# ariana-spalter/human-robot-gym

Measured on AMD Instinct MI355X. Metric: env steps/sec (whole node), ReachHuman+shield 4096 envs, higher is better.
Workload: dtype f64

## Files before the change

human-robot-gym_amd/csrc/hrgym_device.h:

```cpp
#pragma once
#include <hip/hip_runtime.h>
#include <stdint.h>

#include "../../include/hrgym.h"
#include "../../include/hrgym_state.h"

#define NV HRG_NV
#define NARM HRG_NARM
#ifndef HRG_BOX
#define HRG_BOX 0
#endif
#ifndef HRG_LIFT
#define HRG_LIFT 0
#endif
#ifndef HRG_HANDOVER
#define HRG_HANDOVER 0
#endif
#ifndef HRG_STACK
#define HRG_STACK 0
#endif
#ifndef HRG_HULLS
#define HRG_HULLS 0
#endif
#ifndef HRG_HAMMER
#define HRG_HAMMER 0
#endif
#define HRG_BASE_TU (!HRG_BOX && !HRG_STACK && !HRG_HAMMER && !HRG_HULLS)
#define HRG_POSE_TABLE ((!HRG_BOX && !HRG_STACK && !HRG_HAMMER) || HRG_LIFT)
#define HRG_POSE_HCAP 0
#define HRG_POSE_SITE (6 * HRG_NHB)
#define HRG_POSE_ROOT (HRG_POSE_SITE + 3 * HRG_NHJ)
#define HRG_POSE_DIM (HRG_POSE_ROOT + 3)
#define NVT HRG_NVT
#if HRG_HAMMER
#define NVS HRG_NV_HAMMER
#define NCON_DYN HRG_NCON_DYN_HAMMER
#define HM_OB NV
#define HM_ON (NV + 6)
#define HM_OH (NV + 8)
#elif HRG_STACK
#define NVS HRG_NV_STACK
#define NCON_DYN HRG_NCON_DYN_STACK
#define NCUBE HRG_NCUBE
#elif HRG_BOX
#define NVS NVT
#define NCON_DYN HRG_NCON_DYN_BOX
#else
#define NVS NV
#define NCON_DYN HRG_NCON_DYN
#endif
#define BODY_BOX 100
#define DI __device__ __forceinline__
#ifndef HRG_MIN_WAVES
#define HRG_MIN_WAVES 4
#endif
#ifndef HRG_PHASE
#define HRG_PHASE __device__ __forceinline__
#endif
#define PH_DYNTERMS HRG_PHASE
#define PH_HUMAN HRG_PHASE
#define PH_SHIELD HRG_PHASE
#define PH_COLLIDE HRG_PHASE
#define PH_CLASSIFY HRG_PHASE
#define PH_DYNSTEP HRG_PHASE
#define HRG_PI 3.14159265358979323846
#define SIXTH (1.0 / 6.0)

#define GEOM_HUMAN0 HRG_NRCAP
#define GEOM_TABLE (HRG_NRCAP + HRG_NHB)
#define GEOM_FLOOR (GEOM_TABLE + 1)
#define GEOM_BOX (GEOM_FLOOR + 1)

#ifdef HRG_STAMPS
static __device__ unsigned long long g_stamps[32];
static __device__ unsigned long long g_stamps_slow[34];
static __device__ unsigned long long g_slow_thresh = ~0ull;
static __device__ unsigned long long g_envcyc[16384][3];
static __device__ unsigned long long g_envacc[16384][32];
__shared__ unsigned long long g_tbeg;
__shared__ unsigned long long g_acc[32];
__shared__ unsigned long long g_t0;
#define STAMP_NOW(var) do { __builtin_amdgcn_sched_barrier(0); asm volatile("s_memtime %0\n\ts_waitcnt lgkmcnt(0)" : "=s"(var) :: "memory"); __builtin_amdgcn_sched_barrier(0); } while (0)
#define STAMP_DECL
#define STAMP_INIT(lane) do { if ((lane) < 32) g_acc[lane] = 0; unsigned long long _t; STAMP_NOW(_t); g_t0 = _t; g_tbeg = _t; __syncthreads(); } while (0)
#define STAMP(k) do { unsigned long long _t; STAMP_NOW(_t); if (threadIdx.x == 0) { g_acc[k] += _t - g_t0; g_t0 = _t; } } while (0)
#define STAMP_FLUSH(lane)
#define COUNT(k, n) do { if (threadIdx.x == 0) g_acc[k] += (n); } while (0)
#define STAMP_FINAL(lane) do { __syncthreads(); if ((lane) < 32) atomicAdd(&g_stamps[lane], g_acc[lane]); { unsigned long long _te; STAMP_NOW(_te); if (_te - g_tbeg > g_slow_thresh) { if ((lane) < 32) atomicAdd(&g_stamps_slow[lane], g_acc[lane]); if ((lane) == 32) atomicAdd(&g_stamps_slow[32], 1ull); if ((lane) == 33) atomicAdd(&g_stamps_slow[33], _te - g_tbeg); } } if ((lane) < 32 && blockIdx.x < 16384) g_envacc[blockIdx.x][lane] = g_acc[lane]; if ((lane) == 0 && blockIdx.x < 16384) { unsigned long long _t; STAMP_NOW(_t); g_envcyc[blockIdx.x][0] = g_tbeg; g_envcyc[blockIdx.x][1] = _t; unsigned _hw, _xcc; asm volatile("s_getreg_b32 %0, hwreg(HW_REG_HW_ID)\n\ts_getreg_b32 %1, hwreg(HW_REG_XCC_ID)" : "=s"(_hw), "=s"(_xcc)); g_envcyc[blockIdx.x][2] = ((unsigned long long)_xcc << 32) | _hw; } } while (0)
#else
#define STAMP_DECL
#define STAMP_INIT(lane)
#define STAMP(k)
#define STAMP_FLUSH(lane)
#define COUNT(k, n)
#define STAMP_FINAL(lane)
#endif

struct DevModel {
  hrg_model_desc m;
  double Rbase[9];
  double Rq[NV][9];
  int32_t anc_mask[NV];
  int32_t hb_maxdepth;
  double sol_K, sol_Bd;
  double rcap_hl[HRG_NRCAP], hcap_hl[HRG_NHB];
  int32_t hb_njump;
  int32_t hb_jump[4][HRG_NHB];
  int32_t phase_mask;
  hrg_path brake_full;
  double brake_T, brake_ds;
  int32_t hc_n;
  int32_t hc_kind[HRG_NHCAP_MAX], hc_j1[HRG_NHCAP_MAX], hc_j2[HRG_NHCAP_MAX];
  double hc_th[HRG_NHCAP_MAX], hc_v[HRG_NHCAP_MAX], hc_a[HRG_NHCAP_MAX], hc_len[HRG_NHCAP_MAX];
  int32_t n_self;
  int32_t self_i[64], self_j[64];
  int32_t n_chk;
  int32_t chk_i[32], chk_j[32];
  hrg_clip_table clips;
  const double* pose_tab;
  const double* hull_dev;
  double hull_cen[HRG_NHULL][3];
  unsigned long long* mpr_fallback;
};

static inline void hull_centroids(const double* verts, const int32_t* off, double cen[HRG_NHULL][3]) {
  for (int h = 0; h < HRG_NHULL; h++) {
    double s[3] = {0, 0, 0};
    for (int i = off[h]; i < off[h + 1]; i++) for (int a = 0; a < 3; a++) s[a] += verts[3 * i + a];
    for (int a = 0; a < 3; a++) cen[h][a] = s[a] / (double)(off[h + 1] - off[h]);
  }
}

struct Contact {
  int32_t g1, g2, b1, b2;
  double dist, n[3], pos[3];
};

#define ROW_CON0 24
#define ROW_WELD0 (ROW_CON0 + 4 * NCON_DYN)
#if HRG_HAMMER
#define HROW_NFRIC 8
#define HROW_LIM0 9
#define HROW_NLIM 25
#define HROW_EQ0 27
#define HROW_CON0 36
#define HROW_NEQ 9
#define NROW 128
#elif HRG_STACK
#define SROW_WELD0 24
#define SROW_CON0 36
#define NROW HRG_NROW_STACK
#elif HRG_BOX && (HRG_HANDOVER || HRG_LIFT)
#define NROW (ROW_WELD0 + 6)
#else
#define NROW ROW_WELD0
#endif

struct GjkLds { double y[4][3], a[4][3], b[4][3], l[4], lam[4]; int ia[4], ib[4]; };
#if HRG_HULLS && HRG_BOX
struct MprLds { double v[5][3], a[5][3], b[5][3]; };
#endif
struct Lds {
  hrg_env_state st;
  double kR[NV][9], kp[NV][3], Sw[NV][3], Sv[NV][3], vw[NV][3], vv[NV][3];
  double M[NV * NV];
  double bias[NV], a0[NVS], Ma0[NVS], ctrl[NV], qacc[NVS], g[NVS], d[NVS];
#if HRG_BOX
  hrg_box_state bx;
  double bR[9];
  double bMr[9];
  double hand_q[4], hand_off[3];
  int palm_hit, palm_pad;
#if HRG_HANDOVER
  double hcap_keep[HRG_NHB][6];
#endif
#endif
  double act[NV];
  int acc_has_collision, acc_collision_type, acc_failsafe, acc_pad;
#if HRG_HAMMER
  hrg_hammer_state hm;
  double gR[2][9];
  double gc[HRG_HM_NGEOM][3];
  double nail_org[3], nail_axis[3];
  double Mb[64], fb[8];
  double Ihw[9], tauh[3];
  double nsG[(9 + 2 * NCON_DYN) * (10 + 2 * NCON_DYN) / 2];
  Contact con[NCON_DYN];
#elif HRG_STACK
  hrg_stack_state sk;
  Contact con[NCON_DYN];
#elif HRG_BOX
  Contact con[NCON_DYN];
#else
  Contact con[NCON_DYN];
#endif
  union {
    struct {
      double cq[NARM], cv[NARM], ca[NARM], qe[NARM];
      double scap[2][HRG_NSHIELD_RCAP][6];
      double rc[HRG_NSHIELD_RCAP][7];
      hrg_ltt cand;
    };
    struct {
      double F[NV][6];
    };
    struct {
      double hcap[HRG_NHB][6], rcapw[HRG_NRCAP][6];
      int hnear[HRG_NHB];
      double rcen[HRG_NRCAP][3];
#if HRG_HULLS && HRG_BOX
      union { GjkLds gjk; MprLds mpr; };
#elif HRG_HULLS
      GjkLds gjk;
#endif
#if HRG_STACK
      double cR[NCUBE][9];
#endif
    };
#if HRG_HAMMER
    struct {
      double Jc[4 * NCON_DYN + HROW_NEQ][NVS + 1], rg[NROW], rh[NROW];
    };
#elif HRG_STACK
    struct {
      double Jc[4 * NCON_DYN][21], rg[NROW], rh[NROW];
      int con_ca[NCON_DYN], con_cb[NCON_DYN], con_rob[NCON_DYN + 1];
    };
#else
    struct {
      double Jc[4 * NCON_DYN + (HRG_LIFT ? 6 : 0)][NVS + 1], rg[NROW], rh[NROW];
    };
#endif
  };
};

#ifndef HRG_WG_WAVES
#define HRG_WG_WAVES 1
#endif
#if HRG_WG_WAVES > 1
__shared__ Lds g_Lw[HRG_WG_WAVES];
#define g_L (g_Lw[__builtin_amdgcn_readfirstlane((int)(threadIdx.x >> 6))])
#else
__shared__ Lds g_L;
#endif
DI int hrg_lane() { return (int)(threadIdx.x & 63u); }
#define HRG_FAIR_SLOTS (8 * 8 * 2 * 16 * 4 * 8)
struct StepOrder { int32_t* buf; int32_t n; int32_t parity; int32_t* fair; };
DI int hrg_env() { return (int)blockIdx.x * HRG_WG_WAVES + (int)(threadIdx.x >> 6); }
// ... 634 lines not shown
```

human-robot-gym_amd/csrc/hrgym_hip.hip:

```cpp
#include <hip/hip_runtime.h>

#include <cmath>
#include <cstdio>
#include <cstring>
#include <cstdlib>
#include <memory>
#include <string>
#include <vector>

#include "hrgym_kernels.h"

template <class MD>
DI void impedance(const MD& m, double x0, double* imp) {
  const double d0 = m.solimp[0], dmax = m.solimp[1], width = m.solimp[2], mid = m.solimp[3], power = m.solimp[4];
  const double x = fabs(x0) / width;
  double y;
  if (x >= 1) y = 1;
  else if (x <= 0) y = 0;
  else if (x <= mid) { const double u = x / mid; y = u * u * mid; }
  else { const double u = (1 - x) / (1 - mid); y = 1 - u * u * (1 - mid); }
  (void)power;
  *imp = d0 + y * (dmax - d0);
}

// ... 2927 lines not shown
                                                                           int64_t env_id0, hrg_box_state* boxes);
extern "C" __attribute__((visibility("hidden"))) void hrg_lift_launch_step(int n_envs, hipStream_t st, const DevModel* dm, hrg_env_state* states, double* actions, float* obs, float* term_obs,
                                                                            float* reward, uint8_t* done, int32_t* info, double* dbg_r, double* dbg_h, int32_t* dbg_nh, int64_t env_id0,
                                                                            float* scratch_obs, hrg_box_state* boxes, StepOrder ord);
extern "C" __attribute__((visibility("hidden"))) void hrg_lift_launch_reset(int n_envs, hipStream_t st, const DevModel* dm, hrg_env_state* states, const uint8_t* mask, float* obs,
                                                                             int64_t env_id0, hrg_box_state* boxes);
#endif
#if HRG_BASE_TU
extern "C" __attribute__((visibility("hidden"))) void hrg_box_hull_launch_step(int n_envs, hipStream_t st, const DevModel* dm, hrg_env_state* states, double* actions, float* obs, float* term_obs,
                                                                                float* reward, uint8_t* done, int32_t* info, double* dbg_r, double* dbg_h, int32_t* dbg_nh, int64_t env_id0,
                                                                                float* scratch_obs, hrg_box_state* boxes, StepOrder ord);
extern "C" __attribute__((visibility("hidden"))) void hrg_box_hull_launch_reset(int n_envs, hipStream_t st, const DevModel* dm, hrg_env_state* states, const uint8_t* mask, float* obs,
                                                                                 int64_t env_id0, hrg_box_state* boxes);
extern "C" __attribute__((visibility("hidden"))) void hrg_hull_launch_step(int n_envs, hipStream_t st, const DevModel* dm, hrg_env_state* states, double* actions, float* obs, float* term_obs,
                                                                            float* reward, uint8_t* done, int32_t* info, double* dbg_r, double* dbg_h, int32_t* dbg_nh, int64_t env_id0,
                                                                            float* scratch_obs, StepOrder ord);
extern "C" __attribute__((visibility("hidden"))) void hrg_hull_launch_reset(int n_envs, hipStream_t st, const DevModel* dm, hrg_env_state* states, const uint8_t* mask, float* obs,
                                                                             int64_t env_id0);
#endif
#if HRG_HULLS && !HRG_BOX
extern "C" void hrg_hull_launch_step(int n_envs, hipStream_t st, const DevModel* dm, hrg_env_state* states, double* actions, float* obs, float* term_obs, float* reward, uint8_t* done,
                                     int32_t* info, double* dbg_r, double* dbg_h, int32_t* dbg_nh, int64_t env_id0, float* scratch_obs, StepOrder ord) {
  hipLaunchKernelGGL(hrg_step_kernel, HRG_LAUNCH_DIMS(n_envs), 0, st, dm, states, actions, obs, term_obs, reward, done, info, dbg_r, dbg_h, dbg_nh, env_id0, scratch_obs, (ObjState*)nullptr, n_envs, ord);
}
extern "C" void hrg_hull_launch_reset(int n_envs, hipStream_t st, const DevModel* dm, hrg_env_state* states, const uint8_t* mask, float* obs, int64_t env_id0) {
  hipLaunchKernelGGL(hrg_reset_kernel, HRG_LAUNCH_DIMS(n_envs), 0, st, dm, states, mask, obs, env_id0, (ObjState*)nullptr, n_envs);
}
#endif
#if HRG_HAMMER
extern "C" void hrg_hammer_launch_step(int n_envs, hipStream_t st, const DevModel* dm, hrg_env_state* states, double* actions, float* obs, float* term_obs, float* reward, uint8_t* done,
                                       int32_t* info, double* dbg_r, double* dbg_h, int32_t* dbg_nh, int64_t env_id0, float* scratch_obs, hrg_hammer_state* hammers, StepOrder ord) {
  hipLaunchKernelGGL(hrg_step_kernel, HRG_LAUNCH_DIMS(n_envs), 0, st, dm, states, actions, obs, term_obs, reward, done, info, dbg_r, dbg_h, dbg_nh, env_id0, scratch_obs, hammers, n_envs, ord);
}
extern "C" void hrg_hammer_launch_reset(int n_envs, hipStream_t st, const DevModel* dm, hrg_env_state* states, const uint8_t* mask, float* obs, int64_t env_id0, hrg_hammer_state* hammers) {
  hipLaunchKernelGGL(hrg_reset_kernel, HRG_LAUNCH_DIMS(n_envs), 0, st, dm, states, mask, obs, env_id0, hammers, n_envs);
}
#endif
#if HRG_STACK
extern "C" void hrg_stack_launch_step(int n_envs, hipStream_t st, const DevModel* dm, hrg_env_state* states, double* actions, float* obs, float* term_obs, float* reward, uint8_t* done,
                                      int32_t* info, double* dbg_r, double* dbg_h, int32_t* dbg_nh, int64_t env_id0, float* scratch_obs, hrg_stack_state* stacks, StepOrder ord) {
  hipLaunchKernelGGL(hrg_step_kernel, HRG_LAUNCH_DIMS(n_envs), 0, st, dm, states, actions, obs, term_obs, reward, done, info, dbg_r, dbg_h, dbg_nh, env_id0, scratch_obs, stacks, n_envs, ord);
}
extern "C" void hrg_stack_launch_reset(int n_envs, hipStream_t st, const DevModel* dm, hrg_env_state* states, const uint8_t* mask, float* obs, int64_t env_id0, hrg_stack_state* stacks) {
  hipLaunchKernelGGL(hrg_reset_kernel, HRG_LAUNCH_DIMS(n_envs), 0, st, dm, states, mask, obs, env_id0, stacks, n_envs);
}
#endif
#if HRG_BOX
extern "C" void hrg_box_launch_step(int n_envs, hipStream_t st, const DevModel* dm, hrg_env_state* states, double* actions, float* obs, float* term_obs, float* reward, uint8_t* done,
                                    int32_t* info, double* dbg_r, double* dbg_h, int32_t* dbg_nh, int64_t env_id0, float* scratch_obs, hrg_box_state* boxes, StepOrder ord) {
  hipLaunchKernelGGL(hrg_step_kernel, HRG_LAUNCH_DIMS(n_envs), 0, st, dm, states, actions, obs, term_obs, reward, done, info, dbg_r, dbg_h, dbg_nh, env_id0, scratch_obs, boxes, n_envs, ord);
}
extern "C" void hrg_box_launch_reset(int n_envs, hipStream_t st, const DevModel* dm, hrg_env_state* states, const uint8_t* mask, float* obs, int64_t env_id0, hrg_box_state* boxes) {
  hipLaunchKernelGGL(hrg_reset_kernel, HRG_LAUNCH_DIMS(n_envs), 0, st, dm, states, mask, obs, env_id0, boxes, n_envs);
}
#endif

#ifdef HRG_STAMPS
#if HRG_STACK
#define hrg_debug_stamps hrg_debug_stamps_stack
#elif HRG_HAMMER
#define hrg_debug_stamps hrg_debug_stamps_hammer
#elif HRG_BOX && HRG_HULLS
#define hrg_debug_stamps hrg_debug_stamps_box_hull
#elif HRG_HANDOVER
#define hrg_debug_stamps hrg_debug_stamps_ho
#elif HRG_LIFT
#define hrg_debug_stamps hrg_debug_stamps_lift
#elif HRG_BOX
#define hrg_debug_stamps hrg_debug_stamps_box
#elif HRG_HULLS
#define hrg_debug_stamps hrg_debug_stamps_hull
#endif
#if HRG_BASE_TU
extern "C" int hrg_debug_stamps_slow(double* out, unsigned long long thresh, int reset) {
  unsigned long long h[34];
  if (hipMemcpyFromSymbol(h, HIP_SYMBOL(g_stamps_slow), sizeof h) != hipSuccess) return -1;
  for (int i = 0; i < 34; i++) out[i] = (double)h[i];
  if (reset) { memset(h, 0, sizeof h); hipMemcpyToSymbol(HIP_SYMBOL(g_stamps_slow), h, sizeof h); }
  hipMemcpyToSymbol(HIP_SYMBOL(g_slow_thresh), &thresh, sizeof thresh);
  return 0;
}
#endif
extern "C" int hrg_debug_stamps(double* out, int reset) {
  unsigned long long h[32];
  if (hipMemcpyFromSymbol(h, HIP_SYMBOL(g_stamps), sizeof h) != hipSuccess) return -1;
  for (int i = 0; i < 32; i++) out[i] = (double)h[i];
  if (reset) { memset(h, 0, sizeof h); hipMemcpyToSymbol(HIP_SYMBOL(g_stamps), h, sizeof h); }
  return 0;
}
#if HRG_HAMMER
#define hrg_debug_envacc hrg_debug_envacc_hammer
#define hrg_debug_envcyc hrg_debug_envcyc_hammer
#elif HRG_STACK
#define hrg_debug_envacc hrg_debug_envacc_stack
#define hrg_debug_envcyc hrg_debug_envcyc_stack
#elif HRG_BOX && HRG_HULLS
#define hrg_debug_envacc hrg_debug_envacc_box_hull
#define hrg_debug_envcyc hrg_debug_envcyc_box_hull
#elif HRG_HANDOVER
#define hrg_debug_envacc hrg_debug_envacc_ho
#define hrg_debug_envcyc hrg_debug_envcyc_ho
#elif HRG_LIFT
#define hrg_debug_envacc hrg_debug_envacc_lift
#define hrg_debug_envcyc hrg_debug_envcyc_lift
#elif HRG_BOX
#define hrg_debug_envacc hrg_debug_envacc_box
#define hrg_debug_envcyc hrg_debug_envcyc_box
#elif HRG_HULLS
#define hrg_debug_envacc hrg_debug_envacc_hull
#define hrg_debug_envcyc hrg_debug_envcyc_hull
#endif
#if 1
extern "C" int hrg_debug_envacc(unsigned long long* out, int n) { return hipMemcpyFromSymbol(out, HIP_SYMBOL(g_envacc), sizeof(unsigned long long) * 32 * n) == hipSuccess ? 0 : -1; }
extern "C" int hrg_debug_envcyc(unsigned long long* out, int n) { return hipMemcpyFromSymbol(out, HIP_SYMBOL(g_envcyc), sizeof(unsigned long long) * 3 * n) == hipSuccess ? 0 : -1; }
#endif
#endif

#if HRG_BASE_TU

static thread_local std::string g_err;
static int fail(int code, const std::string& msg) { g_err = msg; return code; }
#define HIPCHK(x)                                                                                         \
  do {                                                                                                    \
    hipError_t _e = (x);                                                                                  \
    if (_e != hipSuccess) return fail(HRG_ERR_HIP, std::string(#x) + ": " + hipGetErrorString(_e));        \
  } while (0)

struct hrg_batch {
  int device = 0;
  int32_t n_envs = 0;
  int64_t env_id0 = 0;
  DevModel* d_model = nullptr;
  double* d_frames = nullptr;
  double* d_pose = nullptr;
  size_t pose_bytes = 0;
  double* d_hull = nullptr;
  bool hulls = false;
  unsigned long long* d_mpr_fallback = nullptr;
  hrg_env_state* d_states = nullptr;
  double* d_rcaps = nullptr;
  double* d_hcaps = nullptr;
  int32_t* d_nh = nullptr;
  float* d_scratch_obs = nullptr;
  hrg_box_state* d_boxes = nullptr;
  hrg_stack_state* d_stacks = nullptr;
  hrg_hammer_state* d_hammers = nullptr;
  int32_t* d_order = nullptr;
  int32_t parity = 0;
  int32_t task = HRG_TASK_REACH;
  bool timing = false;
  bool taps = false;
  std::vector<std::pair<hipEvent_t, hipEvent_t>> events;
  std::vector<std::pair<hipEvent_t, hipEvent_t>> pool;
};

static int32_t* fair_table(int device) {
  static int32_t* tab[64] = {nullptr};
  if (device < 0 || device >= 64) return nullptr;
  if (!tab[device]) {
    int32_t* p = nullptr;
    if (hipMalloc(&p, sizeof(int32_t) * HRG_FAIR_SLOTS) != hipSuccess) return nullptr;
    if (hipMemset(p, 0, sizeof(int32_t) * HRG_FAIR_SLOTS) != hipSuccess) { hipFree(p); return nullptr; }
    tab[device] = p;
  }
  return tab[device];
}

static bool hrg_task_uses_pose_table(int task) { return task == HRG_TASK_REACH || task == HRG_TASK_LIFTING; }

// ... 498 lines not shown
```

human-robot-gym_amd/csrc/hrgym_kernels.h:

```cpp
#pragma once
#include "hrgym_device.h"
#if HRG_HULLS
#include "hrgym_hull.h"
#endif

DI void robot_chain_fk(const DevModel* __restrict__ dm_, int lane, bool shield_on) {
  const ModelPtr dm = uniform_model(dm_);
  Lds& L = g_L;
  double* sc = &L.rc[0][0];
  if (lane < 3 * NARM && (lane >= 2 * NARM || shield_on)) {
    const int cfg = lane / NARM, i = lane - NARM * cfg;
    const double q = cfg == 0 ? L.cq[i] : (cfg == 1 ? L.qe[i] : L.st.qpos[i]);
    double sn, cs;
    sincos_small(q, &sn, &cs);
    sc[2 * lane] = sn; sc[2 * lane + 1] = cs;
  }
  wave_sync();
  if (lane < 9 && (lane >= 6 || shield_on)) {
    const auto& m = dm->m;
    const int cfg = lane / 3, row = lane - 3 * cfg;
    double r0 = dm->Rbase[3 * row], r1 = dm->Rbase[3 * row + 1], r2 = dm->Rbase[3 * row + 2];
    double p = m.base_pos[row];
#pragma unroll 1
    for (int i = 0; i < NARM; i++) {
      const double sn = sc[2 * (NARM * cfg + i)], cs = sc[2 * (NARM * cfg + i) + 1];
      p += r0 * m.body_pos[i][0] + r1 * m.body_pos[i][1] + r2 * m.body_pos[i][2];
      double n0 = 0, n1 = 0, n2 = 0;
      {
        const double ra[3] = {r0, r1, r2};
#pragma unroll
        for (int a = 0; a < 3; a++) {
          const double c0 = dm->Rq[i][3 * a], c1 = dm->Rq[i][3 * a + 1], c2 = dm->Rq[i][3 * a + 2];
          n0 += ra[a] * (cs * c0 + sn * c1);
          n1 += ra[a] * (cs * c1 - sn * c0);
          n2 += ra[a] * c2;
        }
      }
      r0 = n0; r1 = n1; r2 = n2;
      if (cfg == 2) {
        L.kR[i][3 * row] = r0; L.kR[i][3 * row + 1] = r1; L.kR[i][3 * row + 2] = r2;
        L.kp[i][row] = p;
      } else {
        L.scap[cfg][i][row] = p + (r0 * m.scap_p1[i][0] + r1 * m.scap_p1[i][1] + r2 * m.scap_p1[i][2]);
        L.scap[cfg][i][3 + row] = p + (r0 * m.scap_p2[i][0] + r1 * m.scap_p2[i][1] + r2 * m.scap_p2[i][2]);
        if (i == NARM - 1) {
          L.scap[cfg][NARM][row] = p + (r0 * m.scap_p1[NARM][0] + r1 * m.scap_p1[NARM][1] + r2 * m.scap_p1[NARM][2]);
          L.scap[cfg][NARM][3 + row] = p + (r0 * m.scap_p2[NARM][0] + r1 * m.scap_p2[NARM][1] + r2 * m.scap_p2[NARM][2]);
        }
      }
    }
    if (cfg == 2) {
#pragma unroll 1
      for (int f = 0; f < HRG_NFINGER; f++) {
        const int i = NARM + f;
        double l[3] = {0, 0, 0};
        {
          const double ra[3] = {r0, r1, r2};
#pragma unroll
          for (int a = 0; a < 3; a++)
#pragma unroll
            for (int b = 0; b < 3; b++) l[b] += ra[a] * dm->Rq[i][3 * a + b];
        }
        double pf = p + (r0 * m.body_pos[i][0] + r1 * m.body_pos[i][1] + r2 * m.body_pos[i][2]);
        const double axw = l[0] * m.jnt_axis[i][0] + l[1] * m.jnt_axis[i][1] + l[2] * m.jnt_axis[i][2];
        pf += axw * L.st.qpos[i];
        L.kR[i][3 * row] = l[0]; L.kR[i][3 * row + 1] = l[1]; L.kR[i][3 * row + 2] = l[2];
        L.kp[i][row] = pf;
      }
    }
  }
  wave_sync();
}

PH_DYNTERMS void robot_dynamics_terms(const DevModel* __restrict__ dm_, int lane) {
  const ModelPtr dm = uniform_model(dm_);
  Lds& L = g_L;
  const auto& m = dm->m;
  double bI[10];
  double Sw[3] = {0, 0, 0}, Sv[3] = {0, 0, 0};
  if (lane < NV) {
    const int i = lane;
    const double* R = L.kR[i];
    double axw[3], t[3], c[3];
    m3mulv(axw, R, m.jnt_axis[i]);
    if (i < NARM) { v3cpy(Sw, axw); v3cross(Sv, L.kp[i], axw); }
    else v3cpy(Sv, axw);
    v3cpy(L.Sw[i], Sw); v3cpy(L.Sv[i], Sv);
    m3mulv(t, R, m.body_com[i]);
    v3add(c, L.kp[i], t);
    const auto* I = m.body_inertia[i];
    const double Ib[9] = {I[0], I[3], I[4], I[3], I[1], I[5], I[4], I[5], I[2]};
    double T[9];
    m3mul(T, R, Ib);
    const double Iw[6] = {v3dot(T, R), v3dot(T + 3, R + 3), v3dot(T + 6, R + 6), v3dot(T, R + 3), v3dot(T, R + 6), v3dot(T + 3, R + 6)};
    sinertia_body(bI, m.body_mass[i], c, Iw);
  } else {
#pragma unroll
    for (int a = 0; a < 10; a++) bI[a] = 0.0;
  }
  const int i = lane < NV ? lane : 0;
  {
    double cc[10];
#pragma unroll
    for (int a = 0; a < 10; a++) cc[a] = subtree_sum(bI[a], lane);
    double n[3], f[3];
    sinertia_mul(n, f, cc, Sw, Sv);
    if (lane < NV) {
#pragma unroll
      for (int a = 0; a < 3; a++) { L.F[i][a] = n[a]; L.F[i][3 + a] = f[a]; }
    }
  }
  __builtin_amdgcn_sched_barrier(0);
  {
    double vw[3], vv[3], aw[3], av[3];
    {
      double jw[3], jv[3];
      const double qd = lane < NV ? L.st.qvel[i] : 0.0;
      v3scl(jw, Sw, qd);
      v3scl(jv, Sv, qd);
      for (int a = 0; a < 3; a++) { vw[a] = chain_prefix(jw[a], lane); vv[a] = chain_prefix(jv[a], lane); }
      double t1[3], t2[3], t3[3];
      v3cross(t1, vw, jw);
      v3cross(t2, vw, jv);
      v3cross(t3, vv, jw);
      for (int a = 0; a < 3; a++) { aw[a] = chain_prefix(t1[a], lane); av[a] = chain_prefix(t2[a] + t3[a], lane) - m.gravity[a]; }
    }
    if (lane < NV) { v3cpy(L.vw[i], vw); v3cpy(L.vv[i], vv); }
    __builtin_amdgcn_sched_barrier(0);
    double fn[3], ff[3];
    {
      double n1[3], f1[3];
      sinertia_mul(n1, f1, bI, aw, av);
      double n2[3], f2[3], t1[3], t2[3], t3[3];
      sinertia_mul(n2, f2, bI, vw, vv);
      v3cross(t1, vw, n2);
      v3cross(t2, vv, f2);
      v3cross(t3, vw, f2);
#pragma unroll
      for (int a = 0; a < 3; a++) { fn[a] = n1[a] + t1[a] + t2[a]; ff[a] = f1[a] + t3[a]; }
    }
    __builtin_amdgcn_sched_barrier(0);
    double gm = 0;
#pragma unroll
    for (int a = 0; a < 3; a++) gm += Sw[a] * subtree_sum(fn[a], lane) + Sv[a] * subtree_sum(ff[a], lane);
    if (lane < NV) L.bias[i] = gm;
  }
  wave_sync();
  {
    const int i = lane >> 3, j = lane & 7;
    double v = 0;
    if ((dm->anc_mask[j] >> i) & 1) v = v3dot(L.Sw[i], &L.F[j][0]) + v3dot(L.Sv[i], &L.F[j][3]);
// ... 419 lines not shown
  fs2.s0 = uniform_f64(fs2.s0); fs2.v0 = uniform_f64(fs2.v0); fs2.a0 = uniform_f64(fs2.a0); fs2.k = uniform_f64(fs2.k);
  for (int a = 0; a < 3; a++) { fs2.dur[a] = uniform_f64(fs2.dur[a]); fs2.jerk[a] = uniform_f64(fs2.jerk[a]); }
  STAMP(11);
  if (shield_on && lane < NARM) {
    double qn, q1, q2, qv;
    ltt_eval2(Lp, lane, s1, se, &qn, &q1, &q2, &qv);
    L.qe[lane] = qv;
    s.des_q[lane] = qn; s.des_v[lane] = q1 * v1; s.des_a[lane] = q1 * a1 + q2 * v1 * v1;
  }
  wave_sync();
  STAMP(12);
  robot_chain_fk(dm_, lane, shield_on);
  STAMP(13);
  int safe = 1;
  if (shield_on) {
    const double sdiff = se - ps;
    double rc_hl = 0;
    if (lane < HRG_NSHIELD_RCAP) {
      const int c = lane;
      double d[3], l1, l2;
      v3sub(d, &L.scap[0][c][0], &L.scap[1][c][0]); l1 = v3norm(d);
      v3sub(d, &L.scap[0][c][3], &L.scap[1][c][3]); l2 = v3norm(d);
      for (int a = 0; a < 6; a++) L.rc[c][a] = 0.5 * (L.scap[0][c][a] + L.scap[1][c][a]);
      L.rc[c][6] = m.scap_r[c] + m.secure_radius + 0.5 * (l1 > l2 ? l1 : l2) + m.scap_alpha[c] * sdiff * sdiff / 8.0;
      double hv[3];
      for (int a = 0; a < 3; a++) hv[a] = 0.5 * (L.rc[c][3 + a] - L.rc[c][a]);
      rc_hl = fsqrt(v3dot(hv, hv));
      L.scap[0][c][0] = rc_hl;
      if (dbg_r) for (int a = 0; a < 7; a++) dbg_r[((size_t)e * HRG_NSHIELD_RCAP + c) * 7 + a] = L.rc[c][a];
    }
    wave_sync();
    double rbl[3], rbh[3];
    {
      double bl[3], bh[3];
      if (lane < HRG_NSHIELD_RCAP) {
        const double rr = L.rc[lane][6];
        for (int a = 0; a < 3; a++) { const double p1 = L.rc[lane][a], p2 = L.rc[lane][3 + a]; bl[a] = (p1 < p2 ? p1 : p2) - rr; bh[a] = (p1 > p2 ? p1 : p2) + rr; }
      } else for (int a = 0; a < 3; a++) { bl[a] = 1e300; bh[a] = -1e300; }
      for (int a = 0; a < 3; a++) { rbh[a] = lane_value<0>(row16_max(bh[a])); rbl[a] = -lane_value<0>(row16_max(-bl[a])); }
    }
    const int nh = dm->hc_n;
    int mdl = -1;
    double c1[3] = {0, 0, 0}, c2[3] = {0, 0, 0}, r = 0, hc[3] = {0, 0, 0}, hl = 0;
    bool near_robot = false;
    if (lane < nh) {
      const int kind = dm->hc_kind[lane], j1 = dm->hc_j1[lane], j2 = dm->hc_j2[lane];
      const double Td = dt + Tb + m.delay;
      if (kind == 0) {
        double va[3], vb[3];
        const double idt = have_vel ? 1.0 / (t - s.meas_prev_t) : 0.0;
        for (int a = 0; a < 3; a++) {
          va[a] = (s.human_site[j1][a] - s.meas_prev[j1][a]) * idt;
          vb[a] = (s.human_site[j2][a] - s.meas_prev[j2][a]) * idt;
        }
        const double base = 0.5 * dm->hc_a[lane] * Td * Td + m.meas_err_pos + m.meas_err_vel * Td;
        const double r1 = v3norm(va) * Td * 0.5 + base, r2 = v3norm(vb) * Td * 0.5 + base;
        v3madd(c1, s.human_site[j1], va, 0.5 * Td);
        v3madd(c2, s.human_site[j2], vb, 0.5 * Td);
        r = (r1 > r2 ? r1 : r2) + dm->hc_th[lane];
        mdl = 0;
      } else if (kind == 2) {
        v3cpy(c1, s.human_site[j1]);
        v3cpy(c2, s.human_site[j1]);
        r = dm->hc_len[lane] + dm->hc_th[lane] + m.meas_err_pos + dm->hc_v[lane] * Td;
        mdl = 2;
      } else {
        v3cpy(c1, s.human_site[j1]);
        v3cpy(c2, s.human_site[j2]);
        r = dm->hc_th[lane] + m.meas_err_pos + dm->hc_v[lane] * Td;
        mdl = kind == 1 ? 1 : 2;
      }
      double hh[3];
      for (int a = 0; a < 3; a++) { hc[a] = 0.5 * (c1[a] + c2[a]); hh[a] = 0.5 * (c2[a] - c1[a]); }
      hl = fsqrt(v3dot(hh, hh));
      double d2b = 0;
      for (int a = 0; a < 3; a++) { const double ee = hc[a] < rbl[a] ? rbl[a] - hc[a] : (hc[a] > rbh[a] ? hc[a] - rbh[a] : 0.0); d2b += ee * ee; }
      near_robot = d2b <= (hl + r + 1e-9) * (hl + r + 1e-9);
      if (dbg_h) {
        double* o = dbg_h + ((size_t)e * HRG_NHCAP_MAX + lane) * 7;
        o[0] = c1[0]; o[1] = c1[1]; o[2] = c1[2]; o[3] = c2[0]; o[4] = c2[1]; o[5] = c2[2]; o[6] = r;
      }
    }
    if (dbg_nh && lane == 0) dbg_nh[e] = nh;
    bool all_hit = true;
#pragma unroll 1
    for (int mm = 0; mm < 3 && all_hit; mm++) {
      if (mm == 0 && !have_vel) continue;
      const bool mine = mdl == mm && near_robot;
      bool hit = false;
      if (__any(mine)) {
#pragma unroll 1
        for (int c = 0; c < HRG_NSHIELD_RCAP; c++) {
          bool close = false;
          const double rr = L.rc[c][6] + r;
          if (mine) {
            double rcn[3], dc[3];
            for (int a = 0; a < 3; a++) rcn[a] = 0.5 * (L.rc[c][a] + L.rc[c][3 + a]);
            v3sub(dc, rcn, hc);
            const double reach = L.scap[0][c][0] + hl + rr + 1e-9;
            close = !(v3dot(dc, dc) > reach * reach);
          }
          if (!__any(close)) continue;
          if (close) { double x1[3], x2[3]; if (seg_seg(&L.rc[c][0], &L.rc[c][3], c1, c2, x1, x2) < rr * rr) hit = true; }
          if (__any(hit)) break;
        }
      }
      all_hit = __any(hit);
    }
    safe = !all_hit;
  }
  wave_sync();
  STAMP(14);
  for (int k = lane; k < HRG_NHJ * 3; k += 64) (&s.meas_prev[0][0])[k] = (&s.human_site[0][0])[k];
  s.meas_prev_t = t;
  if (s.n_meas < 2) s.n_meas = s.n_meas + 1;
  if (safe) {
    if (use_cand) {
      double* dst = (double*)&s.ltt;
      const double* src = (const double*)&L.cand;
      for (int k = lane; k < (int)(sizeof(hrg_ltt) / sizeof(double)); k += 64) dst[k] = src[k];
      s.new_goal = 0;
    }
    s.path_s = s1; s.path_v = v1; s.path_a = a1;
    s.safe_path = fs2;
  } else {
    const double k = s.safe_path.k + 1.0;
    s.safe_path.k = k;
    double ns, nv, na;
    const hrg_path spc = s.safe_path;
    const double vend = pfl ? path_vend(&spc) : m.failsafe_sdot;
    path_eval(&s.safe_path, k * dt, vend, &ns, &nv, &na);
    if (use_cand && s.path_v <= vend + 1e-9 && fabs(s.path_a) <= 1e-9) {
      const double adv = ns - s.path_s;
      double* dst = (double*)&s.ltt;
      const double* src = (const double*)&L.cand;
      for (int q = lane; q < (int)(sizeof(hrg_ltt) / sizeof(double)); q += 64) dst[q] = src[q];
      s.new_goal = 0;
      ns = adv;
      hrg_path sp;
      path_plan(&sp, ns, nv, na, vend, m.path_amax, m.path_jmax);
      s.safe_path = sp;
    }
    s.path_s = ns; s.path_v = nv; s.path_a = na;
  }
  s.is_safe = safe;
  wave_sync();
  if (lane < NARM && !(shield_on && safe)) {
    double qq, q1, q2;
    ltt_eval(&s.ltt, lane, s.path_s, &qq, &q1, &q2);
    s.des_q[lane] = qq; s.des_v[lane] = q1 * s.path_v; s.des_a[lane] = q1 * s.path_a + q2 * s.path_v * s.path_v;
  }
  wave_sync();
  STAMP(15);
}

DI void shield_reset(const DevModel* __restrict__ , int lane) {
  Lds& L = g_L;
  hrg_env_state& s = L.st;
  if (lane < NARM) {
    const double q = s.qpos[lane];
    s.ltt.q0[lane] = q; s.ltt.qT[lane] = q;
    s.des_q[lane] = q; s.new_goal_q[lane] = q; s.goal_qpos[lane] = q;
  }
  s.is_safe = 1;
}

#if HRG_STACK || HRG_HAMMER || HRG_LIFT
#define BB_TIE 1e-9
struct BBContact { double pos[3], n[3], dist; };
#define BB_WORK 152
DI int box_box2(const double* pa, const double* Ra, const double* ha, const double* pb, const double* Rb, const double* hb, BBContact* out, double* T) {
  double (*A)[3] = (double (*)[3])(T + 72), (*B)[3] = (double (*)[3])(T + 81), (*C)[3] = (double (*)[3])(T + 90), (*AC)[3] = (double (*)[3])(T + 99);
  double t[3], ta[3], tb[3];
  v3sub(t, pb, pa);
  for (int i = 0; i < 3; i++) for (int k = 0; k < 3; k++) { A[i][k] = Ra[3 * k + i]; B[i][k] = Rb[3 * k + i]; }
  for (int i = 0; i < 3; i++) { ta[i] = v3dot(t, A[i]); tb[i] = v3dot(t, B[i]); for (int j = 0; j < 3; j++) { C[i][j] = v3dot(A[i], B[j]); AC[i][j] = fabs(C[i][j]); } }
  double sf = -1e300, se = -1e300;
  int bf = 0, be = -1;
  for (int i = 0; i < 3; i++) {
    const double s_ = fabs(ta[i]) - (ha[i] + hb[0] * AC[i][0] + hb[1] * AC[i][1] + hb[2] * AC[i][2]);
    if (s_ > 0) return 0;
    if (s_ > sf + BB_TIE) { sf = s_; bf = i; }
  }
  for (int j = 0; j < 3; j++) {
    const double s_ = fabs(tb[j]) - (hb[j] + ha[0] * AC[0][j] + ha[1] * AC[1][j] + ha[2] * AC[2][j]);
    if (s_ > 0) return 0;
    if (s_ > sf + BB_TIE) { sf = s_; bf = 3 + j; }
  }
#pragma unroll 1
  for (int ij = 0; ij < 9; ij++) {
    const int i = ij / 3, j = ij - 3 * i, i1 = (i + 1) % 3, i2 = (i + 2) % 3, j1 = (j + 1) % 3, j2 = (j + 2) % 3;
    const double l2 = 1.0 - C[i][j] * C[i][j];
    if (l2 < 1e-12) continue;
    const double l = fsqrt(l2);
    const double tl = ta[i2] * C[i1][j] - ta[i1] * C[i2][j];
// ... 811 lines not shown
```

Measured before the change: 4.511 million.

## Parallelize shield FK capsule/finger stages and compact human-robot pair checks across lanes

Robot FK now stores per-link frames for all three configurations in a union with the dynamics scratch space. A second lane-parallel pass then computes shield capsule endpoints and finger frames, which were previously done serially inside the 3-lane-per-config chain loop. The human-vs-robot capsule collision loop compacts active human capsules into an LDS list and spreads (human, robot-capsule) pairs over all 64 lanes using shuffles, instead of looping over robot capsules with sparse lane use. This adds an extra wave sync and shuffle traffic, and it reuses LDS through a union, so it depends on those lifetimes not overlapping.

Measured after the change: 4.576 million (median of 6 runs). +1.4%, better.

```diff
diff --git a/human-robot-gym_amd/csrc/hrgym_device.h b/human-robot-gym_amd/csrc/hrgym_device.h
--- a/human-robot-gym_amd/csrc/hrgym_device.h
+++ b/human-robot-gym_amd/csrc/hrgym_device.h
@@ -72,21 +72,22 @@
 #define GEOM_BOX (GEOM_FLOOR + 1)
 
 #ifdef HRG_STAMPS
-static __device__ unsigned long long g_stamps[32];
+#define HRG_NSTAMP 40
+static __device__ unsigned long long g_stamps[HRG_NSTAMP];
 static __device__ unsigned long long g_stamps_slow[34];
 static __device__ unsigned long long g_slow_thresh = ~0ull;
 static __device__ unsigned long long g_envcyc[16384][3];
 static __device__ unsigned long long g_envacc[16384][32];
 __shared__ unsigned long long g_tbeg;
-__shared__ unsigned long long g_acc[32];
+__shared__ unsigned long long g_acc[HRG_NSTAMP];
 __shared__ unsigned long long g_t0;
 #define STAMP_NOW(var) do { __builtin_amdgcn_sched_barrier(0); asm volatile("s_memtime %0\n\ts_waitcnt lgkmcnt(0)" : "=s"(var) :: "memory"); __builtin_amdgcn_sched_barrier(0); } while (0)
 #define STAMP_DECL
-#define STAMP_INIT(lane) do { if ((lane) < 32) g_acc[lane] = 0; unsigned long long _t; STAMP_NOW(_t); g_t0 = _t; g_tbeg = _t; __syncthreads(); } while (0)
+#define STAMP_INIT(lane) do { if ((lane) < HRG_NSTAMP) g_acc[lane] = 0; unsigned long long _t; STAMP_NOW(_t); g_t0 = _t; g_tbeg = _t; __syncthreads(); } while (0)
 #define STAMP(k) do { unsigned long long _t; STAMP_NOW(_t); if (threadIdx.x == 0) { g_acc[k] += _t - g_t0; g_t0 = _t; } } while (0)
 #define STAMP_FLUSH(lane)
 #define COUNT(k, n) do { if (threadIdx.x == 0) g_acc[k] += (n); } while (0)
-#define STAMP_FINAL(lane) do { __syncthreads(); if ((lane) < 32) atomicAdd(&g_stamps[lane], g_acc[lane]); { unsigned long long _te; STAMP_NOW(_te); if (_te - g_tbeg > g_slow_thresh) { if ((lane) < 32) atomicAdd(&g_stamps_slow[lane], g_acc[lane]); if ((lane) == 32) atomicAdd(&g_stamps_slow[32], 1ull); if ((lane) == 33) atomicAdd(&g_stamps_slow[33], _te - g_tbeg); } } if ((lane) < 32 && blockIdx.x < 16384) g_envacc[blockIdx.x][lane] = g_acc[lane]; if ((lane) == 0 && blockIdx.x < 16384) { unsigned long long _t; STAMP_NOW(_t); g_envcyc[blockIdx.x][0] = g_tbeg; g_envcyc[blockIdx.x][1] = _t; unsigned _hw, _xcc; asm volatile("s_getreg_b32 %0, hwreg(HW_REG_HW_ID)\n\ts_getreg_b32 %1, hwreg(HW_REG_XCC_ID)" : "=s"(_hw), "=s"(_xcc)); g_envcyc[blockIdx.x][2] = ((unsigned long long)_xcc << 32) | _hw; } } while (0)
+#define STAMP_FINAL(lane) do { __syncthreads(); if ((lane) < HRG_NSTAMP) atomicAdd(&g_stamps[lane], g_acc[lane]); { unsigned long long _te; STAMP_NOW(_te); if (_te - g_tbeg > g_slow_thresh) { if ((lane) < 32) atomicAdd(&g_stamps_slow[lane], g_acc[lane]); if ((lane) == 32) atomicAdd(&g_stamps_slow[32], 1ull); if ((lane) == 33) atomicAdd(&g_stamps_slow[33], _te - g_tbeg); } } if ((lane) < 32 && blockIdx.x < 16384) g_envacc[blockIdx.x][lane] = g_acc[lane]; if ((lane) == 0 && blockIdx.x < 16384) { unsigned long long _t; STAMP_NOW(_t); g_envcyc[blockIdx.x][0] = g_tbeg; g_envcyc[blockIdx.x][1] = _t; unsigned _hw, _xcc; asm volatile("s_getreg_b32 %0, hwreg(HW_REG_HW_ID)\n\ts_getreg_b32 %1, hwreg(HW_REG_XCC_ID)" : "=s"(_hw), "=s"(_xcc)); g_envcyc[blockIdx.x][2] = ((unsigned long long)_xcc << 32) | _hw; } } while (0)
 #else
 #define STAMP_DECL
 #define STAMP_INIT(lane)
@@ -162,8 +163,17 @@
 #endif
 struct Lds {
   hrg_env_state st;
-  double kR[NV][9], kp[NV][3], Sw[NV][3], Sv[NV][3], vw[NV][3], vv[NV][3];
-  double M[NV * NV];
+  double kR[NV][9], kp[NV][3];
+  union {
+    struct {
+      double Sw[NV][3], Sv[NV][3], vw[NV][3], vv[NV][3];
+      double M[NV * NV];
+    };
+    struct {
+      double fkR[2][NARM][9], fkp[2][NARM][3];
+      uint8_t hlist[HRG_NHCAP_MAX];
+    };
+  };
   double bias[NV], a0[NVS], Ma0[NVS], ctrl[NV], qacc[NVS], g[NVS], d[NVS];
 #if HRG_BOX
   hrg_box_state bx;
diff --git a/human-robot-gym_amd/csrc/hrgym_hip.hip b/human-robot-gym_amd/csrc/hrgym_hip.hip
--- a/human-robot-gym_amd/csrc/hrgym_hip.hip
+++ b/human-robot-gym_amd/csrc/hrgym_hip.hip
@@ -3033,9 +3033,9 @@
 }
 #endif
 extern "C" int hrg_debug_stamps(double* out, int reset) {
-  unsigned long long h[32];
+  unsigned long long h[HRG_NSTAMP];
   if (hipMemcpyFromSymbol(h, HIP_SYMBOL(g_stamps), sizeof h) != hipSuccess) return -1;
-  for (int i = 0; i < 32; i++) out[i] = (double)h[i];
+  for (int i = 0; i < HRG_NSTAMP; i++) out[i] = (double)h[i];
   if (reset) { memset(h, 0, sizeof h); hipMemcpyToSymbol(HIP_SYMBOL(g_stamps), h, sizeof h); }
   return 0;
 }
diff --git a/human-robot-gym_amd/csrc/hrgym_kernels.h b/human-robot-gym_amd/csrc/hrgym_kernels.h
--- a/human-robot-gym_amd/csrc/hrgym_kernels.h
+++ b/human-robot-gym_amd/csrc/hrgym_kernels.h
@@ -19,6 +19,8 @@
   if (lane < 9 && (lane >= 6 || shield_on)) {
     const auto& m = dm->m;
     const int cfg = lane / 3, row = lane - 3 * cfg;
+    double* const fR = cfg == 2 ? &L.kR[0][0] : &L.fkR[cfg][0][0];
+    double* const fp = cfg == 2 ? &L.kp[0][0] : &L.fkp[cfg][0][0];
     double r0 = dm->Rbase[3 * row], r1 = dm->Rbase[3 * row + 1], r2 = dm->Rbase[3 * row + 2];
     double p = m.base_pos[row];
 #pragma unroll 1
@@ -37,36 +39,34 @@
         }
       }
       r0 = n0; r1 = n1; r2 = n2;
-      if (cfg == 2) {
-        L.kR[i][3 * row] = r0; L.kR[i][3 * row + 1] = r1; L.kR[i][3 * row + 2] = r2;
-        L.kp[i][row] = p;
-      } else {
-        L.scap[cfg][i][row] = p + (r0 * m.scap_p1[i][0] + r1 * m.scap_p1[i][1] + r2 * m.scap_p1[i][2]);
-        L.scap[cfg][i][3 + row] = p + (r0 * m.scap_p2[i][0] + r1 * m.scap_p2[i][1] + r2 * m.scap_p2[i][2]);
-        if (i == NARM - 1) {
-          L.scap[cfg][NARM][row] = p + (r0 * m.scap_p1[NARM][0] + r1 * m.scap_p1[NARM][1] + r2 * m.scap_p1[NARM][2]);
-          L.scap[cfg][NARM][3 + row] = p + (r0 * m.scap_p2[NARM][0] + r1 * m.scap_p2[NARM][1] + r2 * m.scap_p2[NARM][2]);
-        }
-      }
-    }
-    if (cfg == 2) {
-#pragma unroll 1
-      for (int f = 0; f < HRG_NFINGER; f++) {
-        const int i = NARM + f;
-        double l[3] = {0, 0, 0};
-        {
-          const double ra[3] = {r0, r1, r2};
+      fR[9 * i + 3 * row] = r0; fR[9 * i + 3 * row + 1] = r1; fR[9 * i + 3 * row + 2] = r2;
+      fp[3 * i + row] = p;
+    }
+  }
+  wave_sync();
+  if (lane < 2 * HRG_NSHIELD_RCAP * 3 ? shield_on : lane < 2 * HRG_NSHIELD_RCAP * 3 + 3 * HRG_NFINGER) {
+    const auto& m = dm->m;
+    if (lane < 2 * HRG_NSHIELD_RCAP * 3) {
+      const int cfg = lane / (3 * HRG_NSHIELD_RCAP), cr = lane - 3 * HRG_NSHIELD_RCAP * cfg, c = cr / 3, row = cr - 3 * c, i = c < NARM ? c : NARM - 1;
+      const double r0 = L.fkR[cfg][i][3 * row], r1 = L.fkR[cfg][i][3 * row + 1], r2 = L.fkR[cfg][i][3 * row + 2], p = L.fkp[cfg][i][row];
+      L.scap[cfg][c][row] = p + (r0 * m.scap_p1[c][0] + r1 * m.scap_p1[c][1] + r2 * m.scap_p1[c][2]);
+      L.scap[cfg][c][3 + row] = p + (r0 * m.scap_p2[c][0] + r1 * m.scap_p2[c][1] + r2 * m.scap_p2[c][2]);
+    } else {
+      const int fr = lane - 2 * HRG_NSHIELD_RCAP * 3, f = fr / 3, row = fr - 3 * f, i = NARM + f;
+      const double r0 = L.kR[NARM - 1][3 * row], r1 = L.kR[NARM - 1][3 * row + 1], r2 = L.kR[NARM - 1][3 * row + 2], p = L.kp[NARM - 1][row];
+      double l[3] = {0, 0, 0};
+      {
+        const double ra[3] = {r0, r1, r2};
 #pragma unroll
-          for (int a = 0; a < 3; a++)
+        for (int a = 0; a < 3; a++)
 #pragma unroll
-            for (int b = 0; b < 3; b++) l[b] += ra[a] * dm->Rq[i][3 * a + b];
-        }
-        double pf = p + (r0 * m.body_pos[i][0] + r1 * m.body_pos[i][1] + r2 * m.body_pos[i][2]);
-        const double axw = l[0] * m.jnt_axis[i][0] + l[1] * m.jnt_axis[i][1] + l[2] * m.jnt_axis[i][2];
-        pf += axw * L.st.qpos[i];
-        L.kR[i][3 * row] = l[0]; L.kR[i][3 * row + 1] = l[1]; L.kR[i][3 * row + 2] = l[2];
-        L.kp[i][row] = pf;
-      }
+          for (int b = 0; b < 3; b++) l[b] += ra[a] * dm->Rq[i][3 * a + b];
+      }
+      double pf = p + (r0 * m.body_pos[i][0] + r1 * m.body_pos[i][1] + r2 * m.body_pos[i][2]);
+      const double axw = l[0] * m.jnt_axis[i][0] + l[1] * m.jnt_axis[i][1] + l[2] * m.jnt_axis[i][2];
+      pf += axw * L.st.qpos[i];
+      L.kR[i][3 * row] = l[0]; L.kR[i][3 * row + 1] = l[1]; L.kR[i][3 * row + 2] = l[2];
+      L.kp[i][row] = pf;
     }
   }
   wave_sync();
@@ -652,26 +652,46 @@
       }
     }
     if (dbg_nh && lane == 0) dbg_nh[e] = nh;
+    STAMP(14);
+    COUNT(33, 1);
+#ifdef HRG_STAMPS
+    { const int n0 = __popcll(__ballot(mdl == 0 && near_robot)), n1 = __popcll(__ballot(mdl == 1 && near_robot)), n2 = __popcll(__ballot(mdl == 2 && near_robot)); COUNT(36, n0); COUNT(37, n1); COUNT(38, n2); }
+#endif
+    const uint64_t lt = lane == 0 ? 0ull : (~0ull >> (64 - lane));
     bool all_hit = true;
 #pragma unroll 1
     for (int mm = 0; mm < 3 && all_hit; mm++) {
       if (mm == 0 && !have_vel) continue;
+      COUNT(39, 1);
       const bool mine = mdl == mm && near_robot;
+      const uint64_t mmask = __ballot(mine);
       bool hit = false;
-      if (__any(mine)) {
+      if (mmask) {
+        if (mine) L.hlist[__popcll(mmask & lt)] = lane;
+        wave_sync();
+        const int n_pairs = HRG_NSHIELD_RCAP * __popcll(mmask);
 #pragma unroll 1
-        for (int c = 0; c < HRG_NSHIELD_RCAP; c++) {
+        for (int q0 = 0; q0 < n_pairs; q0 += 64) {
+          COUNT(34, 1);
+          const int q = q0 + lane;
+          const bool valid = q < n_pairs;
+          const int k = valid ? q / HRG_NSHIELD_RCAP : 0, c = valid ? q - HRG_NSHIELD_RCAP * k : 0;
+          const int src = L.hlist[k];
+          double p1[3], p2[3], pc[3];
+          for (int a = 0; a < 3; a++) { p1[a] = __shfl(c1[a], src, 64); p2[a] = __shfl(c2[a], src, 64); pc[a] = __shfl(hc[a], src, 64); }
+          const double pr = __shfl(r, src, 64), phl = __shfl(hl, src, 64);
           bool close = false;
-          const double rr = L.rc[c][6] + r;
-          if (mine) {
+          const double rr = L.rc[c][6] + pr;
+          if (valid) {
             double rcn[3], dc[3];
             for (int a = 0; a < 3; a++) rcn[a] = 0.5 * (L.rc[c][a] + L.rc[c][3 + a]);
-            v3sub(dc, rcn, hc);
-            const double reach = L.scap[0][c][0] + hl + rr + 1e-9;
+            v3sub(dc, rcn, pc);
+            const double reach = L.scap[0][c][0] + phl + rr + 1e-9;
             close = !(v3dot(dc, dc) > reach * reach);
           }
           if (!__any(close)) continue;
-          if (close) { double x1[3], x2[3]; if (seg_seg(&L.rc[c][0], &L.rc[c][3], c1, c2, x1, x2) < rr * rr) hit = true; }
+          COUNT(35, 1);
+          if (close) { double x1[3], x2[3]; if (seg_seg(&L.rc[c][0], &L.rc[c][3], p1, p2, x1, x2) < rr * rr) hit = true; }
           if (__any(hit)) break;
         }
       }
@@ -680,7 +700,7 @@
     safe = !all_hit;
   }
   wave_sync();
-  STAMP(14);
+  STAMP(32);
   for (int k = lane; k < HRG_NHJ * 3; k += 64) (&s.meas_prev[0][0])[k] = (&s.human_site[0][0])[k];
   s.meas_prev_t = t;
   if (s.n_meas < 2) s.n_meas = s.n_meas + 1;
```
